# datastax/jvector

Measured on AMD Instinct MI355X. Metric: QPS@recall10>=0.95 (10Mx768); distances/sec as % HBM roofline, higher is better.
Workload: dtype f32

## Files before the change

### jvector_amd/csrc/cabi.cpp

```cpp
#include <algorithm>
#include <cmath>
#include <cstring>
#include <mutex>

#include "jv_device.h"
#include "jv_internal.h"
#include "gs_params.h"
#include "../../include/jvector_formats.h"

namespace jv {

static thread_local char g_err[1024] = "";

void set_error(const char *fmt, ...)
{
    va_list ap;
    va_start(ap, fmt);
    vsnprintf(g_err, sizeof(g_err), fmt, ap);
    va_end(ap);
}
void clear_error() { g_err[0] = 0; }

int Buffer::reserve(size_t bytes)
{
// ... 238 lines not shown
    ctx->d_gs_visited.release();
    ctx->d_gs_spill.release();
    ctx->d_gs_out.release();
    ctx->d_gs_mask.release();
    ctx->d_gs_big.release();
    ctx->d_nvq_q.release();
    ctx->d_gs_extra.release();
    ctx->d_gs_ubr.release();
    ctx->d_bq_work.release();
    ctx->d_bin_work.release();
    ctx->d_bin_cand.release();
    ctx->d_rd_counts.release();
    for (auto &e : ctx->prof_pending) {
        (void)hipEventDestroy(e.start);
        (void)hipEventDestroy(e.stop);
    }
    for (auto &e : ctx->prof_free) (void)hipEventDestroy(e);
    if (ctx->owns_stream) (void)hipStreamDestroy(ctx->stream);
    delete ctx;
    return JV_OK;
}

int jv_hip_ctx_sync(jv_ctx *ctx)
{
    JV_REQUIRE(ctx, "ctx is NULL");
    JV_HIP_CHECK(hipStreamSynchronize(ctx->stream));
    return JV_OK;
}

void *jv_hip_ctx_stream(jv_ctx *ctx) { return ctx ? (void *)ctx->stream : nullptr; }

static int prof_resolve(jv_ctx *ctx)
{
    if (ctx->prof_pending.empty()) return JV_OK;
    JV_HIP_CHECK(hipStreamSynchronize(ctx->stream));
    for (auto &e : ctx->prof_pending) {
        float ms = 0.0f;
        if (hipEventElapsedTime(&ms, e.start, e.stop) == hipSuccess) {
            ctx->prof_ms[e.region] += ms;
            ctx->prof_count[e.region] += 1;
        } else {
            (void)hipGetLastError();
        }
        ctx->prof_free.push_back(e.start);
        ctx->prof_free.push_back(e.stop);
    }
    ctx->prof_pending.clear();
    return JV_OK;
}

int jv_hip_ctx_profile(jv_ctx *ctx, int enable)
{
    clear_error();
    JV_REQUIRE(ctx, "ctx is NULL");
    JV_TRY(use_device(ctx->device));
    JV_TRY(prof_resolve(ctx));
    for (int r = 0; r < R_COUNT; ++r) {
        ctx->prof_ms[r] = 0.0;
        ctx->prof_count[r] = 0;
    }
    ctx->profiling = enable != 0;
    return JV_OK;
}

int jv_hip_ctx_profile_read(jv_ctx *ctx, const char *region, double *total_ms, int64_t *count)
{
    clear_error();
    JV_REQUIRE(ctx && region, "NULL argument");
    static const char *names[R_COUNT] = {"adc", "topk", "exact", "lut", "encode", "norms", "sample", "gsearch", "prune", "adc_exact"};
    int r = -1;
    for (int i = 0; i < R_COUNT; ++i)
        if (strcmp(names[i], region) == 0) r = i;
    JV_REQUIRE(r >= 0, "unknown profile region '%s'", region);
    JV_TRY(use_device(ctx->device));
    JV_TRY(prof_resolve(ctx));
    if (total_ms) *total_ms = ctx->prof_ms[r];
    if (count) *count = ctx->prof_count[r];
    return JV_OK;
}

}
namespace jv {
namespace {
const char *const kOptions[] = {"graph_traversal", "gs_occ", "gs_pair", "gs_pairc", "gs_quad", "rd_table_free", "rd_chunk", "rd_split", "rd_wide_stage", "rd_prof", "rd_square", "bl_insert_alpha_x100", "bl_improve_beam", "bl_ref_order", "bl_sorted_lists", "gs_cand_cap", "gs_waves_per_cu", "gs_vcap_log2", "gs_v1_log2", "gs_prefetch", "gs_generic", "gs_wgx", "gs_wgx_waves", "gs_wgx_slots", "gs_wgx_depth", "gs_wgx_per_cu", "gs_wgx_lut_m", "gs_ubr", "gs_ubrc", "gs_ubr_trim", "gs_plain", "gs_fused_rerank", "gs_defer", "gs_defer_min_level", "adc_bq",
                                "gs_grow", "gs_retry", "gs_prof", "gs_tie_check", "gs_push_log", "gs_push_log_cap", "graph_timing",
                                "no_filter", "quiet", "bq_gs_vcap_log2", "bq_gs_cand_cap", "flat_acc_score_bytes"};
std::string env_name(const char *name)
{
    std::string e = "JVECTOR_HIP_";
    for (const char *c = name; *c; ++c) e.push_back((char)toupper((unsigned char)*c));
    return e;
}
}
bool ctx_opt_is_set(const jv_ctx *ctx, const char *name)
{
    if (ctx && ctx->opts.count(name)) return true;
    return getenv(env_name(name).c_str()) != nullptr;
}
long long ctx_opt(const jv_ctx *ctx, const char *name, long long dflt)
{
    if (ctx) {
        auto it = ctx->opts.find(name);
        if (it != ctx->opts.end()) return it->second;
    }
    const char *e = getenv(env_name(name).c_str());
    if (!e) return dflt;
    if (!strcmp(name, "graph_traversal")) return !strcmp(e, "host") ? JV_TRAVERSAL_HOST : (!strcmp(e, "device") ? JV_TRAVERSAL_DEVICE : dflt);
    return atoll(e);
}
}
extern "C" {

int jv_hip_ctx_set_option(jv_ctx *ctx, const char *name, int64_t value)
{
    clear_error();
    JV_REQUIRE(ctx && name, "ctx_set_option: NULL argument");
    for (const char *k : kOptions)
        if (!strcmp(k, name)) {
            ctx->opts[name] = (long long)value;
            return JV_OK;
        }
    set_error("ctx_set_option: unknown option '%s'", name);
    return JV_ERR_INVALID;
}

int jv_hip_ctx_clear_option(jv_ctx *ctx, const char *name)
{
    clear_error();
    JV_REQUIRE(ctx && name, "ctx_clear_option: NULL argument");
    ctx->opts.erase(name);
    return JV_OK;
}

int jv_hip_ctx_get_stat(jv_ctx *ctx, const char *name, int64_t *out)
{
    clear_error();
    JV_REQUIRE(ctx && name && out, "ctx_get_stat: NULL argument");
    if (strcmp(name, "experimental_build") == 0) {
#ifdef JV_EXPERIMENTAL
        *out = 1;
#else
        *out = 0;
#endif
        return JV_OK;
    }
    if (strcmp(name, "rd_tests") == 0 || strcmp(name, "rd_pairs") == 0) {
        *out = 0;
        if (ctx->d_rd_counts.ptr) {
            unsigned long long h[2] = {0, 0};
            JV_TRY(use_device(ctx->device));
            JV_HIP_CHECK(hipStreamSynchronize(ctx->stream));
            JV_HIP_CHECK(hipMemcpy(h, ctx->d_rd_counts.ptr, sizeof(h), hipMemcpyDeviceToHost));
            *out = (int64_t)h[name[3] == 't' ? 0 : 1];
        }
        return JV_OK;
    }
    auto it = ctx->stats.find(name);
    *out = it == ctx->stats.end() ? 0 : (int64_t)it->second;
    return JV_OK;
}

int jv_hip_ctx_reset_stats(jv_ctx *ctx)
{
    clear_error();
    JV_REQUIRE(ctx, "ctx_reset_stats: NULL argument");
    ctx->stats.clear();
    return JV_OK;
// ... 1068 lines not shown
```

### jvector_amd/csrc/graph_search.cpp

```cpp
#include <algorithm>
#include <atomic>
#include <chrono>
#include <condition_variable>
#include <cstdlib>
#include <functional>
#include <memory>
#include <unordered_map>
#include <mutex>
#include <thread>

#include "gs_host.h"
#include "gs_params.h"
#include "jv_internal.h"

namespace jv {
constexpr long long kGsUbrDefault = 1;
constexpr long long kGsUbrcDefault = 1;


class HostPool {
public:
    explicit HostPool(int nthreads) : n_(nthreads)
    {
        for (int t = 1; t < n_; ++t) threads_.emplace_back([this, t] { worker(t); });
    }
    ~HostPool()
    {
        {
            std::lock_guard<std::mutex> lk(m_);
            stop_.store(true);
            awake_ = true;
        }
        cv_.notify_all();
        gen_.fetch_add(1, std::memory_order_release);
        for (auto &th : threads_) th.join();
    }
    int size() const { return n_; }
    void begin()
    {
        {
            std::lock_guard<std::mutex> lk(m_);
            awake_ = true;
        }
        cv_.notify_all();
    }
    void end()
    {
        std::lock_guard<std::mutex> lk(m_);
        awake_ = false;
    }
    void parallel_for(int n, const std::function<void(int, int)> &fn)
    {
        if (n_ == 1 || n < 2 * n_) {
            fn(0, n);
            return;
        }
        fn_ = &fn;
        total_ = n;
        done_.store(0, std::memory_order_relaxed);
        gen_.fetch_add(1, std::memory_order_release);
        run_chunk(0);
        while (done_.load(std::memory_order_acquire) != n_ - 1) cpu_relax();
    }

private:
    static inline void cpu_relax() { __builtin_ia32_pause(); }
    void run_chunk(int t)
    {
        const int per = (total_ + n_ - 1) / n_;
        const int lo = t * per, hi = std::min(total_, lo + per);
        if (lo < hi) (*fn_)(lo, hi);
    }
    void worker(int t)
    {
        uint64_t seen = 0;
        for (;;) {
            {
                std::unique_lock<std::mutex> lk(m_);
                cv_.wait(lk, [&] { return awake_ || stop_.load(); });
            }
            if (stop_.load()) return;
            long idle = 0;
            for (;;) {
                const uint64_t g = gen_.load(std::memory_order_acquire);
                if (g != seen) {
                    seen = g;
                    if (stop_.load()) return;
                    run_chunk(t);
                    done_.fetch_add(1, std::memory_order_release);
                    idle = 0;
                    continue;
                }
                cpu_relax();
                if (++idle > 4096) {
                    idle = 0;
                    bool aw;
// ... 1023 lines not shown

    return rerank_stage(ctx, pool, l, vectors, vsf, kvsf, Q, topK, opt, ses, fin, q_visited, q_expanded, q_expanded_base, out_ids, out_scores, stats);
}

static int ensure_device_graph(jv_ctx *ctx, jv_graph *g)
{
    std::lock_guard<std::mutex> lk(g->dev_mu);
    if (g->dev_ready) {
        JV_REQUIRE(g->dev_device == ctx->device, "graph: device mirror lives on device %d, search runs on device %d",
                   g->dev_device, ctx->device);
        return JV_OK;
    }
    g->free_mirror();
    g->dev_device = ctx->device;
    g->dev.resize((size_t)g->entry_level + 1);
    auto upload = [&](int32_t **dst, const int32_t *src, size_t n) -> int {
        JV_HIP_CHECK(hipMalloc((void **)dst, sizeof(int32_t) * std::max<size_t>(n, 1)));
        JV_HIP_CHECK(hipMemcpy(*dst, src, sizeof(int32_t) * n, hipMemcpyHostToDevice));
        return JV_OK;
    };
    auto build = [&]() -> int {
        for (int lv = 0; lv <= g->entry_level; ++lv) {
            const jv_graph::Level &L = g->levels[lv];
            jv_graph::DevLevel &d = g->dev[lv];
            if (lv == 0 && g->dev_level0) {
                d.nbrs = const_cast<int32_t *>(g->dev_level0);
                continue;
            }
            JV_TRY(upload(&d.nbrs, L.nbrs.data(), L.nbrs.size()));
            if (!L.nodes.empty()) {
                const GsLevelMap m = gs_build_level_map(L.nodes.data(), L.count);
                JV_TRY(upload(&d.hkeys, m.keys.data(), m.keys.size()));
                JV_TRY(upload(&d.hvals, m.vals.data(), m.vals.size()));
                d.hmask = m.mask;
                d.hshift = m.shift;
            }
        }
        return JV_OK;
    };
    const int rc = build();
    if (rc != JV_OK) {
        g->free_mirror();
        return rc;
    }
    g->dev_ready = true;
    return JV_OK;
}

extern "C++" {
namespace jv {
int graph_device_view(jv_ctx *ctx, const jv_graph *g, GsLevel *lv, GraphDeviceView *out)
{
    JV_REQUIRE(ctx && g && lv && out, "graph: NULL argument");
    JV_REQUIRE(g->entry_node >= 0, "graph: no entry node set");
    if (g->entry_level >= GS_MAX_LEVELS) {
        set_error("graph: %d levels, the device traversal takes %d", g->entry_level + 1, GS_MAX_LEVELS);
        return JV_ERR_UNSUPPORTED;
    }
    if (g->levels[0].nbrs.empty() && !g->dev_level0) {
        set_error("graph: level 0 has neither host rows nor a device adjacency");
        return JV_ERR_UNSUPPORTED;
    }
    JV_TRY(ensure_device_graph(ctx, const_cast<jv_graph *>(g)));
    out->n_nodes = g->n_nodes;
    out->entry_node = g->entry_node;
    out->entry_level = g->entry_level;
    out->max_degree = 0;
    for (int l = 0; l <= g->entry_level; ++l) {
        const jv_graph::DevLevel &d = g->dev[l];
        lv[l].nbrs = d.nbrs;
        lv[l].hkeys = d.hkeys;
        lv[l].hvals = d.hvals;
        lv[l].hmask = d.hmask;
        lv[l].hshift = d.hshift;
        lv[l].count = g->levels[l].count;
        lv[l].degree = g->levels[l].degree;
        out->max_degree = std::max(out->max_degree, g->levels[l].degree);
    }
    return JV_OK;
}
}
}

struct DeviceSessionOut {
    float threshold = 0.0f;
    const std::vector<jv_searcher::Call> *history = nullptr;
    int new_rerankK = 0;
    int log_cap = 0;
    std::vector<int32_t> status, base, log_n;
    std::vector<int64_t> stats;
    std::vector<long long> log;
};

static int graph_search_device(jv_ctx *ctx, const jv_graph *g, jv_luts *l, const jv_codes *codes, const jv_fused *fused,
                               const jv_vectors *vectors, const float *queries, int Q, jv_vsf vsf, int topK, int rerankK,
                               int32_t *out_ids, float *out_scores, int64_t *stats, AcceptMask host_accept, AcceptMask dev_accept,
                               DeviceSessionOut *so = nullptr)
{
    const jv_decoder_kind kind = fused ? JV_DECODER_FUSED : JV_DECODER_PQ;
    JV_TRY(luts_prepare(ctx, l, queries, Q, vsf, kind, false));
    const int kvsf = to_kernel_vsf(vsf);
    if (vsf == JV_COSINE) {
        JV_TRY(ensure_code_norms(ctx, const_cast<jv_codes *>(codes)));
        if (fused) JV_TRY(ensure_fused_norms(ctx, const_cast<jv_fused *>(fused)));
    }
    JV_TRY(ensure_device_graph(ctx, const_cast<jv_graph *>(g)));
    const jv_pq *pq = l->pq;

    const bool generic = !graph_search_device_specialised(pq, codes, fused) || ctx_opt(ctx, "gs_generic", 0) != 0;
    const int occ = ctx_opt(ctx, "gs_occ", generic ? 4 : 2) >= 4 ? 4 : 2;
    bool pair = occ == 2 && !generic && ctx_opt(ctx, "gs_pair", 1) != 0;
    for (int lv = 0; lv <= g->entry_level; ++lv) pair = pair && g->levels[lv].degree <= 32;
    pair = pair && pq->M <= 96;
    const long long wgx_opt = ctx_opt(ctx, "gs_wgx", -1);
    bool one_wave_tuned = false;
    for (const char *o : {"gs_vcap_log2", "gs_v1_log2", "gs_grow", "gs_retry", "gs_occ", "gs_pair", "gs_cand_cap", "gs_waves_per_cu", "gs_prefetch", "gs_prof"})
        one_wave_tuned = one_wave_tuned || ctx_opt_is_set(ctx, o);
    bool wgx = !so && !generic && graph_search_wgx_supported(pq->M) &&
               (wgx_opt > 0 || (wgx_opt < 0 && !one_wave_tuned && Q <= 4 * ctx->num_cus));
    for (int lv = 0; lv <= g->entry_level; ++lv) wgx = wgx && g->levels[lv].degree <= 64;
    const int wgx_log = std::min(512, std::max(256, 4 * rerankK));
    int wgx_kps = 32;
    for (int lv = 0; lv <= g->entry_level; ++lv)
        if (g->levels[lv].degree > 32) wgx_kps = 64;
    const int wgx_waves = std::max(2, std::min(8, (int)ctx_opt(ctx, "gs_wgx_waves", 8)));
    const int wgx_slots = std::max(2, std::min((int)GX_MAX_SLOTS, (int)ctx_opt(ctx, "gs_wgx_slots", 16)));
    int evict_cap = GS_EVICT_CAP;
    const int wgx_cand_cap = 256;
    const int wgx_per_cu = std::max(1, std::min(4, (int)ctx_opt(ctx, "gs_wgx_per_cu", 1)));
    const size_t wgx_budget = ctx->lds_per_block / (size_t)wgx_per_cu - (wgx_per_cu > 1 ? 256 : 512);
    auto wgx_bytes = [&](int lg, int lm) { return graph_search_wgx_lds_bytes(pq->D, rerankK, wgx_cand_cap, evict_cap, lg, wgx_slots, wgx_kps, wgx_log, lm); };
    int wgx_lut_m = (int)ctx_opt(ctx, "gs_wgx_lut_m", 0);
    if (wgx) {
        const int idb = gs_idbits(g->n_nodes);
        int min_v1 = 0;
        for (int lg = 12; lg >= 8 && min_v1 == 0; --lg)
            if (gs_v1_fits(lg, idb)) min_v1 = lg;
        if (wgx_lut_m <= 0) {
            wgx_lut_m = pq->M;
            while (wgx_lut_m > 16 && wgx_bytes(min_v1, wgx_lut_m) > wgx_budget) wgx_lut_m -= 16;
        }
        wgx_lut_m = std::max(16, std::min(pq->M, wgx_lut_m / 16 * 16));
        wgx = wgx_bytes(0, wgx_lut_m) <= wgx_budget;
    }
    if (wgx) pair = false;
    bool pairc = occ == 2 && !so && !wgx && !pair && !generic && !fused && pq->M <= 192 && ctx_opt(ctx, "gs_pair", 1) != 0 &&
                 ctx_opt(ctx, "gs_pairc", 1) != 0;
    for (int lv = 0; lv <= g->entry_level; ++lv) pairc = pairc && g->levels[lv].degree <= 64;
    const bool ubr = !so && !wgx && (pair || (pairc && ctx_opt(ctx, "gs_ubrc", kGsUbrcDefault) != 0)) && occ == 2 && !dev_accept.bits && !dev_accept.exclude &&
                     ctx_opt(ctx, "gs_ubr", kGsUbrDefault) != 0 && graph_search_ubr_supported(pq->M, kvsf)
#ifdef JV_EXPERIMENTAL
                     && ctx_opt(ctx, "gs_quad", 0) == 0
#endif
        ;
    const int pair_M = (pair || pairc) ? pq->M : 0;
    int cand_cap = wgx ? wgx_cand_cap : std::max(128, (int)ctx_opt(ctx, "gs_cand_cap", (occ == 4 ? 512 : ((pair || pairc) ? 256 : 1024)))) & ~63;
    while (!wgx && cand_cap > 256 && graph_search_lds_bytes(pq->D, rerankK, cand_cap, pair_M, evict_cap) > 40 * 1024) cand_cap = (cand_cap / 2) & ~63;
    const int idbits = gs_idbits(g->n_nodes);
    const int want_per_cu = 4 * occ;
    const size_t lut_lds = so ? gs_session_lds_bytes() : 0;
    const size_t lds_budget = (160 * 1024) / (size_t)want_per_cu - 256 - lut_lds;
    int v1_log2 = 0;
    if (wgx) {
        const long long pin = ctx_opt(ctx, "gs_v1_log2", ctx_opt_is_set(ctx, "gs_vcap_log2") ? 0 : -1);
        for (int lg = pin > 0 ? (int)pin : 14; lg >= (pin > 0 ? (int)pin : 8) && pin != 0; --lg) {
            if (!gs_v1_fits(lg, idbits)) continue;
            if (wgx_bytes(lg, wgx_lut_m) <= wgx_budget) {
                v1_log2 = lg;
                break;
            }
        }
    } else {
        const long long pin = ctx_opt(ctx, "gs_v1_log2", ctx_opt_is_set(ctx, "gs_vcap_log2") ? 0 : -1);
        struct Caps { int cand, evict; };
        const int cand_small = std::min(cand_cap, 128);
        const long long left = (long long)lds_budget - (long long)graph_search_lds_bytes(pq->D, rerankK, cand_small, pair_M, 1, 12) + 8;
        const Caps caps[3] = {{cand_cap, evict_cap}, {cand_small, evict_cap}, {cand_small, (int)std::max<long long>(96, std::min<long long>(evict_cap, left / 8))}};
        bool done = false;
        for (int lg = pin > 0 ? (int)pin : 12; lg >= (pin > 0 ? (int)pin : 10) && !done && pin != 0; --lg) {
            if (!gs_v1_fits(lg, idbits)) continue;
            for (const Caps &c : caps) {
                if (ctx_opt_is_set(ctx, "gs_cand_cap") && c.cand != cand_cap) continue;
                if (graph_search_lds_bytes(pq->D, rerankK, c.cand, pair_M, c.evict, lg) <= lds_budget || (pin > 0 && &c == &caps[2])) {
                    v1_log2 = lg;
                    cand_cap = c.cand;
                    evict_cap = c.evict;
                    done = true;
                    break;
                }
            }
        }
    }
    const size_t lds = wgx ? wgx_bytes(v1_log2, wgx_lut_m)
                           : graph_search_lds_bytes(pq->D, rerankK, cand_cap, pair_M, evict_cap, v1_log2) + lut_lds;
    if (lds > ctx->lds_per_block) {
        set_error("graph_search(device): rerankK %d needs %zu bytes of LDS per wave (limit %zu); use the host traversal", rerankK,
                  lds, ctx->lds_per_block);
        return JV_ERR_UNSUPPORTED;
    }
    int per_cu = (int)std::min<size_t>((size_t)want_per_cu, std::max<size_t>(1, (160 * 1024) / (lds + 256)));
    per_cu = std::max(1, (int)ctx_opt(ctx, "gs_waves_per_cu", per_cu));
    if (wgx) per_cu = wgx_per_cu;
    const int workers = std::max(1, std::min(Q, ctx->num_cus * per_cu));
    const int vcap_log2 = std::max(8, std::min(24, (int)ctx_opt(ctx, "gs_vcap_log2", gs_vcap_log2(rerankK))));
    const size_t vcap = (size_t)1 << vcap_log2;
    const size_t v1_slots = v1_log2 > 0 ? ((size_t)1 << v1_log2) : 0;
    const int spill_cap = (int)(vcap / 2 + v1_slots) + 64;
    JV_TRY(ctx->d_gs_visited.reserve(sizeof(int32_t) * vcap * (size_t)workers));
    JV_TRY(ctx->d_gs_spill.reserve(sizeof(long long) * (size_t)spill_cap * (size_t)workers));
    const int big_log2 = std::min(24, vcap_log2 + 3);
    const bool grow_on = ctx_opt_is_set(ctx, "gs_grow") ? ctx_opt(ctx, "gs_grow", 1) != 0 : !ctx_opt_is_set(ctx, "gs_vcap_log2");
    const int big_count = (grow_on && big_log2 > vcap_log2) ? std::max(1, std::min(Q, std::max(64, std::min(2048, Q / 32)))) : 0;
    const int big_spill_cap = (int)(((size_t)1 << big_log2) / 2 + v1_slots) + 64;
    const size_t big_vis_bytes = sizeof(int32_t) * ((size_t)1 << big_log2) * (size_t)big_count;
    const size_t big_spill_off = (big_vis_bytes + 255) & ~(size_t)255;
    const size_t big_ctr_off = (big_spill_off + sizeof(long long) * (size_t)big_spill_cap * (size_t)big_count + 255) & ~(size_t)255;
    if (big_count > 0) {
        JV_TRY(ctx->d_gs_big.reserve(big_ctr_off + 256));
        JV_HIP_CHECK(hipMemsetAsync((char *)ctx->d_gs_big.ptr + big_ctr_off, 0, sizeof(uint32_t), ctx->stream));
    }
    const size_t c1 = (size_t)Q * rerankK;
    size_t off = 0;
    auto carve = [&](size_t bytes) {
        const size_t o = off;
        off = (off + bytes + 255) & ~(size_t)255;
        return o;
    };
    const size_t o_ids = carve(sizeof(int32_t) * c1), o_sc = carve(sizeof(float) * c1), o_qn = carve(sizeof(float) * (size_t)Q);
    const size_t o_stats = carve(sizeof(long long) * 2 * (size_t)Q), o_status = carve(sizeof(int32_t) * (size_t)Q);
    const size_t o_counter = carve(sizeof(uint32_t) * 2);
    const size_t o_qmap = carve(sizeof(int32_t) * (size_t)Q);
    bool gs_prof = !so && ctx_opt(ctx, "gs_prof", 0) != 0;
    if (gs_prof && pairc) {
        if (ctx_opt(ctx, "quiet", 0) == 0)
            fprintf(stderr, "[jv gs prof] the compacted pair form (rows of 33..64 neighbours: the builder's searches) has no phase-clock variant; gs_prof ignored for this launch\n");
        gs_prof = false;
    }
    const size_t o_prof = carve(sizeof(unsigned long long) * 36);
    const bool defer_on = !so && !wgx && ubr && pair && ctx_opt(ctx, "gs_defer", 1) != 0 &&
                          (ctx_opt_is_set(ctx, "gs_defer") || g->defer_off.load(std::memory_order_relaxed) == 0);
    const bool tie_check = !so && vectors != nullptr && rerankK > topK && ctx_opt(ctx, "gs_tie_check", 1) != 0;
    int log_cap = 0;
    if (so || (tie_check && ctx_opt(ctx, "gs_push_log", 1) != 0)) {
        log_cap = so ? std::max(4096, 8 * rerankK) : std::max(256, 4 * rerankK);
        const size_t budget = (size_t)1 << 30;
        if ((size_t)Q * log_cap * sizeof(long long) > budget) log_cap = (int)std::max<size_t>(64, budget / ((size_t)Q * sizeof(long long)));
        if (ctx_opt_is_set(ctx, "gs_push_log_cap")) log_cap = std::max(1, (int)ctx_opt(ctx, "gs_push_log_cap", log_cap));
    }
    const size_t o_log = carve(sizeof(long long) * (size_t)Q * (size_t)log_cap), o_log_n = carve(sizeof(int32_t) * (size_t)Q);
    const size_t o_base = carve(sizeof(int32_t) * (size_t)Q);
    JV_TRY(ctx->d_gs_out.reserve(off));
    char *base = (char *)ctx->d_gs_out.ptr;
    int32_t *d_cand = (int32_t *)(base + o_ids);
    float *d_cand_sc = (float *)(base + o_sc);
    float *d_qnorm = (float *)(base + o_qn);
    long long *d_stats = (long long *)(base + o_stats);
    int32_t *d_status = (int32_t *)(base + o_status);
    uint32_t *d_counter = (uint32_t *)(base + o_counter);
    JV_HIP_CHECK(hipMemsetAsync(d_counter, 0, sizeof(uint32_t), ctx->stream));
    if (gs_prof || ubr) JV_HIP_CHECK(hipMemsetAsync(base + o_prof, 0, sizeof(unsigned long long) * 36, ctx->stream));

    GsParams p{};
    for (int lv = 0; lv <= g->entry_level; ++lv) {
        const jv_graph::DevLevel &d = g->dev[lv];
        p.lv[lv].nbrs = d.nbrs;
        p.lv[lv].hkeys = d.hkeys;
        p.lv[lv].hvals = d.hvals;
        p.lv[lv].hmask = d.hmask;
        p.lv[lv].hshift = d.hshift;
        p.lv[lv].count = g->levels[lv].count;
        p.lv[lv].degree = g->levels[lv].degree;
    }
    p.entry_node = g->entry_node;
    p.entry_level = g->entry_level;
    p.codebooks = pq->d_codebooks;
    p.cq = l->d_queries;
    p.bmag = l->d_bmag;
    p.codes = codes->d_codes;
    p.code_norms = codes->d_norms;
    p.blocks = fused ? fused->d_blocks : nullptr;
    p.fused_norms = fused ? fused->d_norms : nullptr;
    p.D = pq->D;
    p.M = pq->M;
    p.deg0 = g->levels[0].degree;
    p.generic = generic ? 1 : 0;
    p.sub_uniform4 = (generic && pq->uniform && pq->max_size % 4 == 0) ? pq->max_size : 0;
    p.sub_sizes = pq->d_sizes;
    p.sub_offsets = pq->d_offsets;
    p.cb_offsets = reinterpret_cast<const long long *>(pq->d_cb_offsets);
    p.Q = Q;
    p.rerankK = rerankK;
    p.accept = (const unsigned long long *)dev_accept.bits;
    p.accept_stride = dev_accept.stride_words;
    p.exclude = dev_accept.exclude;
    p.visited = (int32_t *)ctx->d_gs_visited.ptr;
    p.vcap_log2 = vcap_log2;
    p.spill = (long long *)ctx->d_gs_spill.ptr;
    p.spill_cap = spill_cap;
    p.cand_cap = cand_cap;
    p.evict_cap = evict_cap;
    p.v1_log2 = v1_log2;
    p.v1_idbits = idbits;
    p.prefetch = (ctx_opt(ctx, "gs_prefetch", 0) != 0 && evict_cap >= 48 && !generic) ? 1 : 0;
    if (ubr) {
        const size_t tab_bytes = (gs_ubr_tab_bytes(pq->M) * (size_t)Q + 255) & ~(size_t)255;
        JV_TRY(ctx->d_gs_ubr.reserve(tab_bytes + sizeof(float) * 4 * (size_t)Q));
        p.ubr = 1;
        p.ubr_tab = (const uint32_t *)ctx->d_gs_ubr.ptr;
        p.ubr_meta = (const float *)((const char *)ctx->d_gs_ubr.ptr + tab_bytes);
        p.ubr_trim = std::max(1, (int)ctx_opt(ctx, "gs_ubr_trim", 16));
        p.ubr_count = (unsigned long long *)(base + o_prof) + 15;
        ProfScope ps(ctx, R_LUT);
        JV_TRY(launch_ubr_tables(ctx->stream, kvsf, pq->d_codebooks, l->d_queries, Q, pq->M, (uint32_t *)ctx->d_gs_ubr.ptr,
                                 (float *)((char *)ctx->d_gs_ubr.ptr + tab_bytes)));
    }
    if (wgx) {
        p.prefetch = 0;
        p.wgx = 1;
        p.wgx_slots = wgx_slots;
        p.wgx_kps = wgx_kps;
        p.wgx_log = wgx_log;
        p.wgx_lut_m = wgx_lut_m;
        p.wgx_depth = (int)ctx_opt(ctx, "gs_wgx_depth", 1);
    }
    auto launch = [&](const GsParams &pp, int w) -> int {
        if (pp.ubr) return launch_graph_search_ubr(ctx->stream, kvsf, pp, w, lds);
        return wgx ? launch_graph_search_wgx(ctx->stream, kvsf, pp, w, 64 * wgx_waves) : launch_graph_search(ctx->stream, kvsf, pp, w, occ);
    };
    if (so) {
        p.session = 1;
        p.threshold = so->threshold;
        p.out_base = (int32_t *)(base + o_base);
        if (so->history && !so->history->empty()) {
            const std::vector<jv_searcher::Call> &h = *so->history;
            const int np = (int)h.size() + 1;
            std::vector<int32_t> off((size_t)(np - 1) * Q + 1);
            size_t total = 0;
            for (int t = 0; t < np - 1; ++t) {
                p.ph_rerankK[t] = h[(size_t)t].rerankK;
                p.ph_threshold[t] = h[(size_t)t].threshold;
                for (int q = 0; q < Q; ++q) {
                    off[(size_t)t * Q + q] = (int32_t)total;
                    total += (size_t)(h[(size_t)t].ev_off[(size_t)q + 1] - h[(size_t)t].ev_off[(size_t)q]);
                }
            }
            off.back() = (int32_t)total;
            p.ph_rerankK[np - 1] = so->new_rerankK;
            p.ph_threshold[np - 1] = so->threshold;
            p.n_phases = np;
            p.ph_Q = Q;
            const size_t off_bytes = (sizeof(int32_t) * off.size() + 15) & ~(size_t)15;
            JV_TRY(ctx->d_gs_extra.reserve(off_bytes + sizeof(long long) * std::max<size_t>(total, 1)));
            JV_HIP_CHECK(hipMemcpyAsync(ctx->d_gs_extra.ptr, off.data(), sizeof(int32_t) * off.size(), hipMemcpyHostToDevice, ctx->stream));
            size_t at = 0;
            for (int t = 0; t < np - 1; ++t) {
                const size_t n = h[(size_t)t].ev_keys.size();
                if (n) JV_HIP_CHECK(hipMemcpyAsync((char *)ctx->d_gs_extra.ptr + off_bytes + sizeof(long long) * at, h[(size_t)t].ev_keys.data(),
                                                   sizeof(long long) * n, hipMemcpyHostToDevice, ctx->stream));
                at += n;
            }
            JV_HIP_CHECK(hipStreamSynchronize(ctx->stream));
            p.ph_extra_off = (const int32_t *)ctx->d_gs_extra.ptr;
            p.ph_extra = (const long long *)((const char *)ctx->d_gs_extra.ptr + off_bytes);
        }
    }
    if (big_count > 0) {
        p.big_visited = (int32_t *)ctx->d_gs_big.ptr;
        p.big_spill = (long long *)((char *)ctx->d_gs_big.ptr + big_spill_off);
        p.big_next = (uint32_t *)((char *)ctx->d_gs_big.ptr + big_ctr_off);
        p.big_count = big_count;
        p.big_log2 = big_log2;
        p.big_spill_cap = big_spill_cap;
    }
    p.pair = pair ? 1 : (pairc ? 2 : 0);
#ifdef JV_EXPERIMENTAL
    p.quad = ctx_opt(ctx, "gs_quad", 0) != 0 ? 1 : 0;
#else
    p.quad = 0;
#endif
    p.out_ids = d_cand;
    p.out_scores = d_cand_sc;
    p.out_stats = d_stats;
    p.out_status = d_status;
    p.next_query = d_counter;
    if (log_cap > 0) {
        p.push_log = (long long *)(base + o_log);
        p.push_log_n = (int32_t *)(base + o_log_n);
        p.push_log_cap = log_cap;
    }
    p.prof = gs_prof ? (unsigned long long *)(base + o_prof) : nullptr;
    p.plain = ctx_opt(ctx, "gs_plain", 1) != 0 ? 1 : 0;
    if (defer_on) {
        p.defer = 1;
        p.defer_count = (unsigned long long *)(base + o_prof) + 33;
        p.defer_min_level = (int)std::max<long long>(1, ctx_opt(ctx, "gs_defer_min_level", 2));
    }
    int rr_rows = 0;
    if (!so && !wgx && ubr && pair && vectors && !vectors->nvq && vectors->D == pq->D && gs_rr_lds_bytes() <= lds && ctx_opt(ctx, "gs_fused_rerank", 1) != 0) {
        if (vsf == JV_COSINE) JV_TRY(ensure_vector_norms(ctx, const_cast<jv_vectors *>(vectors)));
        rr_rows = exact_fused_rows(vectors->d_vecs, vectors->D, l->d_raw_queries, Q, kvsf, rerankK, vectors->d_sqnorm);
    }
    if (rr_rows > 0) {
        if (vsf == JV_COSINE) {
            ProfScope ps(ctx, R_EXACT);
            JV_TRY(launch_query_sqnorms(ctx->stream, l->d_raw_queries, vectors->D, Q, d_qnorm));
        }
        p.rr_vecs = vectors->d_vecs;
        p.rr_queries = l->d_raw_queries;
        p.rr_qnorm = d_qnorm;
        p.rr_vnorm = vectors->d_sqnorm;
        p.rr_n = vectors->count;
        p.rr_rows = rr_rows;
    }
    {
        ProfScope ps(ctx, R_GSEARCH);
        JV_TRY(launch(p, workers));
    }
    std::vector<int32_t> status((size_t)Q);
    std::vector<int> redo;
    size_t n_overflow_first = 0;
    {
        JV_TRY(ctx->h_out.reserve(sizeof(int32_t) * (size_t)Q));
        JV_HIP_CHECK(hipMemcpyAsync(ctx->h_out.ptr, d_status, sizeof(int32_t) * (size_t)Q, hipMemcpyDeviceToHost, ctx->stream));
        unsigned long long ubr_dropped = 0;
        if (ubr) JV_HIP_CHECK(hipMemcpyAsync(&ubr_dropped, base + o_prof + 15 * sizeof(unsigned long long), sizeof(ubr_dropped), hipMemcpyDeviceToHost, ctx->stream));
        unsigned long long defer_counts[3] = {0, 0, 0};
        if (defer_on) JV_HIP_CHECK(hipMemcpyAsync(defer_counts, base + o_prof + 33 * sizeof(unsigned long long), sizeof(defer_counts), hipMemcpyDeviceToHost, ctx->stream));
        JV_HIP_CHECK(hipStreamSynchronize(ctx->stream));
        if (ubr) ctx_stat_add(ctx, "gs_ubr_dropped", (long long)ubr_dropped);
        if (defer_on) {
            ctx_stat_add(ctx, "gs_deferred", (long long)defer_counts[0]);
            ctx_stat_add(ctx, "gs_defer_restarts", (long long)defer_counts[1]);
            if (Q >= 64 && defer_counts[1] * 10 > (unsigned long long)Q && g->defer_off.exchange(1, std::memory_order_relaxed) == 0)
                ctx_stat_add(ctx, "gs_defer_switched_off", 1);
        }
        memcpy(status.data(), ctx->h_out.ptr, sizeof(int32_t) * (size_t)Q);
        for (int q = 0; q < Q; ++q)
            if (status[q] != GS_OK) redo.push_back(q);
        n_overflow_first = redo.size();
    }
    const bool retry = ctx_opt_is_set(ctx, "gs_retry") ? ctx_opt(ctx, "gs_retry", 1) != 0 : !ctx_opt_is_set(ctx, "gs_vcap_log2");
    for (int attempt = 1; attempt <= 2 && !redo.empty() && retry; ++attempt) {
        const int vlog2 = std::min(24, vcap_log2 + 3 * attempt);
        if (vlog2 <= vcap_log2 + 3 * (attempt - 1)) break;
        const size_t vcap2 = (size_t)1 << vlog2;
        const int spill2 = (int)(vcap2 / 2 + v1_slots) + 64;
        const int R = (int)redo.size();
        const int workers2 = std::max(1, std::min<int>({R, workers, (int)(((size_t)512 << 20) / (vcap2 * 12))}));
        JV_TRY(ctx->d_gs_visited.reserve(sizeof(int32_t) * vcap2 * (size_t)workers2));
        JV_TRY(ctx->d_gs_spill.reserve(sizeof(long long) * (size_t)spill2 * (size_t)workers2));
        memcpy(ctx->h_out.ptr, redo.data(), sizeof(int32_t) * (size_t)R);
        JV_HIP_CHECK(hipMemcpyAsync(base + o_qmap, ctx->h_out.ptr, sizeof(int32_t) * (size_t)R, hipMemcpyHostToDevice, ctx->stream));
        JV_HIP_CHECK(hipMemsetAsync(d_counter, 0, sizeof(uint32_t), ctx->stream));
        GsParams p2 = p;
        p2.qmap = (const int32_t *)(base + o_qmap);
        p2.Q = R;
        p2.visited = (int32_t *)ctx->d_gs_visited.ptr;
        p2.vcap_log2 = vlog2;
        p2.spill = (long long *)ctx->d_gs_spill.ptr;
        p2.spill_cap = spill2;
        p2.big_visited = nullptr;
        p2.big_count = 0;
        p2.big_log2 = 0;
        p2.prof = nullptr;
        p2.defer = 0;
        {
            ProfScope ps(ctx, R_GSEARCH);
            JV_TRY(launch(p2, workers2));
        }
        JV_HIP_CHECK(hipStreamSynchronize(ctx->stream));
        JV_HIP_CHECK(hipMemcpyAsync(ctx->h_out.ptr, d_status, sizeof(int32_t) * (size_t)Q, hipMemcpyDeviceToHost, ctx->stream));
        JV_HIP_CHECK(hipStreamSynchronize(ctx->stream));
        memcpy(status.data(), ctx->h_out.ptr, sizeof(int32_t) * (size_t)Q);
        std::vector<int> still;
        for (int q : redo)
            if (status[q] != GS_OK) still.push_back(q);
        redo.swap(still);
    }
    if (gs_prof) {
        unsigned long long h[33];
        JV_HIP_CHECK(hipMemcpyAsync(h, base + o_prof, sizeof(h), hipMemcpyDeviceToHost, ctx->stream));
        JV_HIP_CHECK(hipStreamSynchronize(ctx->stream));
        const double e = (double)std::max<unsigned long long>(h[5], 1);
        fprintf(stderr, "[jv gs prof] clocks/expansion: pop %.0f  result %.0f  row+block+visited %.0f  score %.0f  push %.0f | expansions %llu "
                        "queries %llu  setup+epilogue clocks/query %.0f\n", h[0] / e, h[1] / e, h[2] / e, h[3] / e, h[4] / e, h[5], h[6],
                (double)h[7] / (double)std::max<unsigned long long>(h[6], 1));
        const double fs = (double)std::max<unsigned long long>(h[8] + h[9] + h[10] + h[11], 1);
        {
            const double nq = (double)std::max<unsigned long long>(h[6], 1);
            fprintf(stderr, "[jv gs prof] clocks/query outside the expansion loop: setup %.0f  level transitions %.0f  epilogue %.0f  table build %.0f\n",
                    h[12] / nq, h[13] / nq, h[14] / nq, h[15] / nq);
            fprintf(stderr, "[jv gs prof] levels above 0: %.2f expansions per query, %.0f clocks per query (searchOneLayer + transitions) = %.0f per expansion\n",
                    h[24] / nq, h[25] / nq, (double)h[25] / (double)std::max<unsigned long long>(h[24], 1));
            {
                const double eu = (double)std::max<unsigned long long>(h[24], 1);
                fprintf(stderr, "[jv gs prof] levels above 0, clocks/expansion: pop %.0f  result %.0f  row+visited %.0f  score %.0f  push %.0f | scoring passes %.2f per expansion, %.0f clocks per pass\n",
                        h[26] / eu, h[27] / eu, h[28] / eu, h[29] / eu, h[30] / eu, h[32] / eu, (double)h[31] / (double)std::max<unsigned long long>(h[32], 1));
            }
        }
        if (wgx)
            fprintf(stderr, "[jv gs prof] workgroup form, per expansion: row found in a slot %.3f (of those still being scored at use: %.3f of all)  "
                            "requested at the pop %.3f  rows requested ahead %.3f\n", h[8] / e, h[9] / e, h[10] / e, h[11] / e);
        else if (ubr) {
            fprintf(stderr, "[jv gs prof] register-table bound form, per expansion: bound + staging %.0f clocks  bound + staging + exact scores %.0f clocks  "
                            "trims %.0f clocks | dropped %.2f  exactly scored %.2f neighbours\n", h[8] / e, h[9] / e, h[10] / e, h[15] / e, h[11] / e);
            fprintf(stderr, "[jv gs prof] register-table bound form, per expansion: wait for the row %.0f clocks  scoring rounds %.0f  owner sum + finish %.0f  "
                            "passes %.2f | expansions with <= 4 / <= 8 / <= 16 survivors: %.3f / %.3f / %.3f\n", h[16] / e, h[17] / e, h[18] / e, h[19] / e,
                    h[20] / e, h[21] / e, h[22] / e);
        }
        else
        fprintf(stderr, "[jv gs prof] scored neighbours by fresh count of their expansion: <=8 %.3f  <=16 %.3f  <=24 %.3f  <=32 %.3f\n", h[8] / fs,
                h[9] / fs, h[10] / fs, h[11] / fs);
    }

    if (so) {
        so->status.assign(status.begin(), status.end());
        so->base.resize((size_t)Q);
        so->log_n.resize((size_t)Q);
        so->stats.resize(2 * (size_t)Q);
        JV_HIP_CHECK(hipMemcpyAsync(so->base.data(), base + o_base, sizeof(int32_t) * (size_t)Q, hipMemcpyDeviceToHost, ctx->stream));
        JV_HIP_CHECK(hipMemcpyAsync(so->log_n.data(), base + o_log_n, sizeof(int32_t) * (size_t)Q, hipMemcpyDeviceToHost, ctx->stream));
        JV_HIP_CHECK(hipMemcpyAsync(so->stats.data(), d_stats, sizeof(long long) * 2 * (size_t)Q, hipMemcpyDeviceToHost, ctx->stream));
        JV_HIP_CHECK(hipStreamSynchronize(ctx->stream));
        int longest = 0;
        bool overflowed = false;
        for (int q = 0; q < Q; ++q) {
            overflowed = overflowed || so->log_n[(size_t)q] > log_cap;
            longest = std::max(longest, std::min(so->log_n[(size_t)q], log_cap));
        }
        so->log_cap = overflowed ? -1 : std::max(longest, 1);
        if (!overflowed) {
            so->log.resize((size_t)Q * (size_t)so->log_cap);
            JV_HIP_CHECK(hipMemcpy2DAsync(so->log.data(), sizeof(long long) * (size_t)so->log_cap, base + o_log, sizeof(long long) * (size_t)log_cap,
                                          sizeof(long long) * (size_t)so->log_cap, (size_t)Q, hipMemcpyDeviceToHost, ctx->stream));
            JV_HIP_CHECK(hipStreamSynchronize(ctx->stream));
        }
        ctx_stat_add(ctx, "gs_calls_device", 1);
        ctx_stat_add(ctx, "gs_queries_device", Q);
        ctx_stat_add(ctx, "gs_session_calls_device", 1);
        return JV_OK;
    }
    OutStage oi, osc;
    JV_TRY(stage_out_begin(ctx, out_ids, sizeof(int32_t) * (size_t)Q * topK, ctx->d_scratch2, &oi));
    JV_TRY(stage_out_begin(ctx, out_scores, sizeof(float) * (size_t)Q * topK, ctx->d_scratch3, &osc));
    JV_TRY(ctx->d_scratch.reserve(topk_scratch_bytes(Q, topK)));
    if (vectors && rr_rows > 0) {
        if (rr_rows < rerankK) {
            ProfScope ps(ctx, R_EXACT);
            JV_TRY(launch_exact_gather_tail(ctx->stream, vectors->d_vecs, vectors->count, vectors->D, l->d_raw_queries, Q, kvsf, d_cand, rerankK, rr_rows,
                                            d_cand_sc, d_qnorm, vectors->d_sqnorm));
        }
    } else if (vectors) {
        JV_TRY(rerank_gather(ctx, vectors, l->d_raw_queries, Q, vsf, d_cand, rerankK, d_cand_sc, d_qnorm));
    }
    {
        ProfScope ps(ctx, R_TOPK);
        JV_TRY(launch_topk(ctx->stream, ctx, d_cand_sc, d_cand, Q, rerankK, rerankK, 0, topK, (int32_t *)oi.dev,
                           (float *)osc.dev, ctx->d_scratch.ptr));
    }
    if (tie_check) {
        JV_HIP_CHECK(hipMemsetAsync(d_counter, 0, sizeof(uint32_t) * 2, ctx->stream));
        ProfScope ps(ctx, R_TOPK);
        RtParams rt{};
        rt.cand_sc = d_cand_sc;
        rt.cand_ids = d_cand;
        rt.R = rerankK;
        rt.out_sc = (float *)osc.dev;
        rt.out_ids = (int32_t *)oi.dev;
        rt.K = topK;
        rt.Q = Q;
        rt.push_log = p.push_log;
        rt.push_log_n = p.push_log_n;
        rt.log_cap = p.push_log_cap;
        rt.rerankK = rerankK;
        rt.status = d_status;
        rt.count = d_counter;
        JV_TRY(launch_rerank_ties(ctx->stream, rt));
    }
    JV_TRY(stage_out_end(ctx, oi));
    JV_TRY(stage_out_end(ctx, osc));
    const size_t stats_bytes = stats ? sizeof(long long) * 2 * (size_t)Q : 0;
    JV_TRY(ctx->h_out.reserve(stats_bytes + 64));
    unsigned int *h_ties = (unsigned int *)((char *)ctx->h_out.ptr + stats_bytes);
    h_ties[0] = h_ties[1] = 0;
    if (tie_check) JV_HIP_CHECK(hipMemcpyAsync(h_ties, d_counter, sizeof(uint32_t) * 2, hipMemcpyDeviceToHost, ctx->stream));
    if (stats) {
        long long *h_stats = (long long *)ctx->h_out.ptr;
        JV_HIP_CHECK(hipMemcpyAsync(h_stats, d_stats, sizeof(long long) * 2 * (size_t)Q, hipMemcpyDeviceToHost, ctx->stream));
        JV_HIP_CHECK(hipStreamSynchronize(ctx->stream));
        for (int q = 0; q < Q; ++q) {
            stats[2 * q] = h_stats[2 * q];
            stats[2 * q + 1] = h_stats[2 * q + 1];
        }
    } else {
        JV_HIP_CHECK(hipStreamSynchronize(ctx->stream));
    }
    const size_t n_ties = h_ties[0], n_ties_resolved = h_ties[1];
    if (n_ties > 0) {
        JV_TRY(ctx->h_out.reserve(sizeof(int32_t) * (size_t)Q));
        JV_HIP_CHECK(hipMemcpyAsync(ctx->h_out.ptr, d_status, sizeof(int32_t) * (size_t)Q, hipMemcpyDeviceToHost, ctx->stream));
        JV_HIP_CHECK(hipStreamSynchronize(ctx->stream));
        const int32_t *hs = (const int32_t *)ctx->h_out.ptr;
        for (int q = 0; q < Q; ++q)
            if (hs[q] == GS_RERANK_TIE) redo.push_back(q);
        std::sort(redo.begin(), redo.end());
    }
    ctx_stat_add(ctx, "gs_calls_device", 1);
    ctx_stat_add(ctx, "gs_queries_device", Q);
    ctx_stat_add(ctx, "gs_queries_retried", (long long)n_overflow_first);
    ctx_stat_add(ctx, "gs_ties_resolved_device", (long long)n_ties_resolved);
    ctx_stat_add(ctx, "gs_ties_to_host", (long long)n_ties);
    ctx_stat_add(ctx, "gs_queries_host_fallback", (long long)redo.size());
    ctx_stat_set(ctx, "gs_last_v1_log2", v1_log2);
    ctx_stat_set(ctx, "gs_last_workers_per_cu", per_cu);
    ctx_stat_set(ctx, "gs_last_wgx", wgx ? 1 : 0);
    ctx_stat_set(ctx, "gs_last_ubr", ubr ? 1 : 0);
    ctx_stat_set(ctx, "gs_last_plain", (!wgx && gs_params_plain(p)) ? 1 : 0);
    ctx_stat_set(ctx, "gs_last_rr_rows", rr_rows);
    ctx_stat_set(ctx, "gs_last_pair", pair ? 1 : (pairc ? 2 : 0));
    if (wgx) ctx_stat_add(ctx, "gs_calls_wgx", 1);
    if (ctx_opt(ctx, "graph_timing", 0) != 0)
        fprintf(stderr, "[jv graph_search device] Q=%d workers=%d (x%d/CU, occ %d, pair %d, wgx %d) lds=%zu cand_cap=%d evict_cap=%d v1_log2=%d vcap=%zu overflow=%zu rerank ties=%zu (+%zu to the host) -> host %zu\n", Q,
                workers, per_cu, occ, pair ? 1 : (pairc ? 2 : 0), wgx ? wgx_waves : 0, lds, cand_cap, evict_cap, v1_log2, vcap, n_overflow_first, n_ties_resolved, n_ties, redo.size());
    if (redo.empty()) return JV_OK;

    jv_graph *gm = const_cast<jv_graph *>(g);
    std::unique_lock<std::mutex> loan_lock(gm->dev_mu, std::defer_lock);
    if (g->dev_level0) loan_lock.lock();
    struct Level0Loan {
        jv_graph *g;
        bool active = false;
        ~Level0Loan()
        {
            if (active) {
                g->levels[0].nbrs.clear();
                g->levels[0].nbrs.shrink_to_fit();
// ... 475 lines not shown
```

Baseline: 2.587 million.

## Add lean query preamble kernel replacing LUT preparation in device graph search

Adds a new HIP kernel that, in one pass over the raw queries, writes centered queries, computes per-query centered magnitudes for cosine, and optionally computes query squared norms. Device graph search uses it by default instead of the full luts_prepare path, stages host queries straight to the device, and reuses the kernel-computed query norms so the separate sqnorm launch is skipped. This targets per-call host and device preamble overhead, at the cost of a new code path that marks tables invalid and must match the old preparation exactly.

```diff
diff --git a/jvector_amd/csrc/cabi.cpp b/jvector_amd/csrc/cabi.cpp
--- a/jvector_amd/csrc/cabi.cpp
+++ b/jvector_amd/csrc/cabi.cpp
@@ -344,7 +344,7 @@
 }
 namespace jv {
 namespace {
-const char *const kOptions[] = {"graph_traversal", "gs_occ", "gs_pair", "gs_pairc", "gs_quad", "rd_table_free", "rd_chunk", "rd_split", "rd_wide_stage", "rd_prof", "rd_square", "bl_insert_alpha_x100", "bl_improve_beam", "bl_ref_order", "bl_sorted_lists", "gs_cand_cap", "gs_waves_per_cu", "gs_vcap_log2", "gs_v1_log2", "gs_prefetch", "gs_generic", "gs_wgx", "gs_wgx_waves", "gs_wgx_slots", "gs_wgx_depth", "gs_wgx_per_cu", "gs_wgx_lut_m", "gs_ubr", "gs_ubrc", "gs_ubr_trim", "gs_plain", "gs_fused_rerank", "gs_defer", "gs_defer_min_level", "adc_bq",
+const char *const kOptions[] = {"graph_traversal", "gs_occ", "gs_pair", "gs_pairc", "gs_quad", "rd_table_free", "rd_chunk", "rd_split", "rd_wide_stage", "rd_prof", "rd_square", "bl_insert_alpha_x100", "bl_improve_beam", "bl_ref_order", "bl_sorted_lists", "gs_cand_cap", "gs_waves_per_cu", "gs_vcap_log2", "gs_v1_log2", "gs_prefetch", "gs_generic", "gs_wgx", "gs_wgx_waves", "gs_wgx_slots", "gs_wgx_depth", "gs_wgx_per_cu", "gs_wgx_lut_m", "gs_ubr", "gs_ubrc", "gs_ubr_trim", "gs_plain", "gs_lean_step", "gs_fused_rerank", "gs_defer", "gs_defer_min_level", "adc_bq",
                                 "gs_grow", "gs_retry", "gs_prof", "gs_tie_check", "gs_push_log", "gs_push_log_cap", "graph_timing",
                                 "no_filter", "quiet", "bq_gs_vcap_log2", "bq_gs_cand_cap", "flat_acc_score_bytes"};
 std::string env_name(const char *name)
diff --git a/jvector_amd/csrc/graph_search.cpp b/jvector_amd/csrc/graph_search.cpp
--- a/jvector_amd/csrc/graph_search.cpp
+++ b/jvector_amd/csrc/graph_search.cpp
@@ -12,6 +12,7 @@
 #include "gs_host.h"
 #include "gs_params.h"
 #include "jv_internal.h"
+#include "sp_params.h"
 
 namespace jv {
 constexpr long long kGsUbrDefault = 1;
@@ -1201,6 +1202,49 @@
 }
 }
 
+extern "C++" {
+namespace jv {
+#ifdef __HIP__
+int launch_step_preamble(hipStream_t s, const SpPreParams &p, size_t p_bytes);
+static inline bool step_preamble_present() { return true; }
+#else
+int launch_step_preamble_emulated(hipStream_t s, const SpPreParams &p, size_t p_bytes) __attribute__((weak));
+static inline int launch_step_preamble(hipStream_t s, const SpPreParams &p, size_t p_bytes) { return launch_step_preamble_emulated(s, p, p_bytes); }
+static inline bool step_preamble_present() { return launch_step_preamble_emulated != nullptr; }
+#endif
+}
+}
+
+static int step_stage_queries(jv_ctx *ctx, jv_luts *l, const float *queries, int Q, jv_vsf vsf, jv_decoder_kind kind, const float **raw_out)
+{
+    *raw_out = nullptr;
+    if (!step_preamble_present()) return JV_OK;
+    if (!ctx || !l || !queries || Q <= 0 || Q > l->capacity) return JV_OK;
+    if (vsf != JV_EUCLIDEAN && vsf != JV_DOT_PRODUCT && vsf != JV_COSINE) return JV_OK;
+    const jv_pq *pq = l->pq;
+    if (pq->D < 8 || pq->D % 8 != 0) return JV_OK;
+    const bool block8 = kind != JV_DECODER_FUSED || (pq->uniform && pq->max_size == 8 && pq->D == 8 * pq->M);
+    if (vsf == JV_COSINE && !block8) return JV_OK;
+    const bool dev = is_device_ptr(queries);
+    if (dev && (reinterpret_cast<uintptr_t>(queries) & 15) != 0) return JV_OK;
+    JV_TRY(use_device(ctx->device));
+    l->Q = Q;
+    l->vsf = vsf;
+    l->kind = kind;
+    l->tables_valid = false;
+    if (dev) {
+        *raw_out = queries;
+        return JV_OK;
+    }
+    const size_t qbytes = sizeof(float) * (size_t)Q * pq->D;
+    JV_HIP_CHECK(hipStreamSynchronize(ctx->stream));
+    JV_TRY(ctx->h_in.reserve(qbytes));
+    memcpy(ctx->h_in.ptr, queries, qbytes);
+    JV_HIP_CHECK(hipMemcpyAsync(l->d_raw_queries, ctx->h_in.ptr, qbytes, hipMemcpyHostToDevice, ctx->stream));
+    *raw_out = l->d_raw_queries;
+    return JV_OK;
+}
+
 struct DeviceSessionOut {
     float threshold = 0.0f;
     const std::vector<jv_searcher::Call> *history = nullptr;
@@ -1217,7 +1261,14 @@
                                DeviceSessionOut *so = nullptr)
 {
     const jv_decoder_kind kind = fused ? JV_DECODER_FUSED : JV_DECODER_PQ;
-    JV_TRY(luts_prepare(ctx, l, queries, Q, vsf, kind, false));
+    const float *q_raw = nullptr;
+    if (!so && ctx_opt(ctx, "gs_lean_step", 1) != 0) JV_TRY(step_stage_queries(ctx, l, queries, Q, vsf, kind, &q_raw));
+    const bool lean_pre = q_raw != nullptr;
+    if (!lean_pre) {
+        JV_TRY(luts_prepare(ctx, l, queries, Q, vsf, kind, false));
+        q_raw = l->d_raw_queries;
+    }
+    ctx_stat_set(ctx, "gs_last_lean_step", lean_pre ? 1 : 0);
     const int kvsf = to_kernel_vsf(vsf);
     if (vsf == JV_COSINE) {
         JV_TRY(ensure_code_norms(ctx, const_cast<jv_codes *>(codes)));
@@ -1378,6 +1429,23 @@
     uint32_t *d_counter = (uint32_t *)(base + o_counter);
     JV_HIP_CHECK(hipMemsetAsync(d_counter, 0, sizeof(uint32_t), ctx->stream));
     if (gs_prof || ubr) JV_HIP_CHECK(hipMemsetAsync(base + o_prof, 0, sizeof(unsigned long long) * 36, ctx->stream));
+    const bool pre_qnorm = lean_pre && vsf == JV_COSINE && vectors && vectors->D == l->pq->D;
+    if (lean_pre) {
+        ProfScope ps(ctx, R_LUT);
+        SpPreParams sp{};
+        sp.raw = q_raw;
+        sp.centroid = l->pq->d_centroid;
+        sp.cq = l->d_queries;
+        sp.bmag = vsf == JV_COSINE ? l->d_bmag : nullptr;
+        sp.qnorm = pre_qnorm ? d_qnorm : nullptr;
+        sp.Q = Q;
+        sp.D = l->pq->D;
+        const int rc = launch_step_preamble(ctx->stream, sp, sizeof(sp));
+        if (rc != JV_OK) {
+            set_error("graph_search(device): the query preamble kernel could not be launched (%d)", rc);
+            return rc;
+        }
+    }
 
     GsParams p{};
     for (int lv = 0; lv <= g->entry_level; ++lv) {
@@ -1517,15 +1585,15 @@
     int rr_rows = 0;
     if (!so && !wgx && ubr && pair && vectors && !vectors->nvq && vectors->D == pq->D && gs_rr_lds_bytes() <= lds && ctx_opt(ctx, "gs_fused_rerank", 1) != 0) {
         if (vsf == JV_COSINE) JV_TRY(ensure_vector_norms(ctx, const_cast<jv_vectors *>(vectors)));
-        rr_rows = exact_fused_rows(vectors->d_vecs, vectors->D, l->d_raw_queries, Q, kvsf, rerankK, vectors->d_sqnorm);
+        rr_rows = exact_fused_rows(vectors->d_vecs, vectors->D, q_raw, Q, kvsf, rerankK, vectors->d_sqnorm);
     }
     if (rr_rows > 0) {
-        if (vsf == JV_COSINE) {
+        if (vsf == JV_COSINE && !pre_qnorm) {
             ProfScope ps(ctx, R_EXACT);
-            JV_TRY(launch_query_sqnorms(ctx->stream, l->d_raw_queries, vectors->D, Q, d_qnorm));
+            JV_TRY(launch_query_sqnorms(ctx->stream, q_raw, vectors->D, Q, d_qnorm));
         }
         p.rr_vecs = vectors->d_vecs;
-        p.rr_queries = l->d_raw_queries;
+        p.rr_queries = q_raw;
         p.rr_qnorm = d_qnorm;
         p.rr_vnorm = vectors->d_sqnorm;
         p.rr_n = vectors->count;
@@ -1666,11 +1734,11 @@
     if (vectors && rr_rows > 0) {
         if (rr_rows < rerankK) {
             ProfScope ps(ctx, R_EXACT);
-            JV_TRY(launch_exact_gather_tail(ctx->stream, vectors->d_vecs, vectors->count, vectors->D, l->d_raw_queries, Q, kvsf, d_cand, rerankK, rr_rows,
+            JV_TRY(launch_exact_gather_tail(ctx->stream, vectors->d_vecs, vectors->count, vectors->D, q_raw, Q, kvsf, d_cand, rerankK, rr_rows,
                                             d_cand_sc, d_qnorm, vectors->d_sqnorm));
         }
     } else if (vectors) {
-        JV_TRY(rerank_gather(ctx, vectors, l->d_raw_queries, Q, vsf, d_cand, rerankK, d_cand_sc, d_qnorm));
+        JV_TRY(rerank_gather(ctx, vectors, q_raw, Q, vsf, d_cand, rerankK, d_cand_sc, d_qnorm));
     }
     {
         ProfScope ps(ctx, R_TOPK);
diff --git a/jvector_amd/csrc/k_step.hip b/jvector_amd/csrc/k_step.hip
--- /dev/null
+++ b/jvector_amd/csrc/k_step.hip
@@ -0,0 +1,37 @@
+#include <hip/hip_runtime.h>
+
+#include <cstddef>
+#include <cstdint>
+
+#include "../../include/jvector_hip.h"
+#include "sp_params.h"
+
+#include "gs_wave_hip.h"
+
+#include "sp_body.h"
+
+#define SP_EXPORT __attribute__((visibility("default")))
+
+namespace jv {
+
+template <bool CENTER>
+__global__ __launch_bounds__(64) void step_preamble_kernel(SpPreParams p)
+{
+    __shared__ __attribute__((aligned(16))) float tile[(SP_ROWS + 1) * SP_LS];
+    sp_preamble<CENTER>(p, (int64_t)blockIdx.x, tile);
+}
+
+SP_EXPORT int launch_step_preamble(hipStream_t s, const SpPreParams &p, size_t p_bytes)
+{
+    if (p_bytes != sizeof(SpPreParams) || p.Q < 0 || !p.raw || !p.cq || p.raw == p.cq) return JV_ERR_INVALID;
+    if (p.Q == 0) return JV_OK;
+    const uintptr_t align = reinterpret_cast<uintptr_t>(p.raw) | reinterpret_cast<uintptr_t>(p.cq) | reinterpret_cast<uintptr_t>(p.centroid);
+    if (p.D < 8 || p.D % 8 != 0 || (align & 15) != 0) return JV_ERR_UNSUPPORTED;
+    const dim3 grid((unsigned)((p.Q + SP_ROWS - 1) / SP_ROWS));
+    if (p.centroid) hipLaunchKernelGGL(step_preamble_kernel<true>, grid, dim3(64), 0, s, p);
+    else hipLaunchKernelGGL(step_preamble_kernel<false>, grid, dim3(64), 0, s, p);
+    if (hipGetLastError() != hipSuccess) return JV_ERR_HIP;
+    return JV_OK;
+}
+
+}
diff --git a/jvector_amd/csrc/sp_body.h b/jvector_amd/csrc/sp_body.h
--- /dev/null
+++ b/jvector_amd/csrc/sp_body.h
@@ -0,0 +1,86 @@
+#pragma once
+
+#include <cstdint>
+
+#include "sp_params.h"
+
+namespace jv {
+
+template <bool CENTER>
+GS_FN void sp_preamble(const SpPreParams &p, int64_t wave, float *tile )
+{
+    constexpr int CH = SP_CH, LS = SP_LS;
+    const int lane = gs_lane();
+    const int seg = (lane & 15) * 4;
+    const int sub = lane >> 4;
+    const int64_t q0 = wave * SP_ROWS;
+    const int D = p.D;
+    const int nc = (D + CH - 1) / CH;
+    SpF4 r[16], cen{0.0f, 0.0f, 0.0f, 0.0f};
+    auto issue = [&](int c) {
+        const int col = c * CH + seg < D ? c * CH + seg : 0;
+#pragma unroll
+        for (int k = 0; k < 16; ++k) {
+            const int64_t q = q0 + 4 * k + sub < p.Q ? q0 + 4 * k + sub : (int64_t)p.Q - 1;
+            r[k] = *reinterpret_cast<const SpF4 *>(p.raw + q * D + col);
+        }
+        if (CENTER) cen = *reinterpret_cast<const SpF4 *>(p.centroid + col);
+    };
+    issue(0);
+    float mag = 0.0f, nrm = 0.0f;
+    for (int c = 0; c < nc; ++c) {
+        const bool in = c * CH + seg < D;
+#pragma unroll
+        for (int k = 0; k < 16; ++k) {
+            *reinterpret_cast<SpF4 *>(tile + (4 * k + sub) * LS + seg) = r[k];
+            const int64_t q = q0 + 4 * k + sub;
+            if (q < p.Q && in) {
+                SpF4 o{r[k].x, r[k].y, r[k].z, r[k].w};
+                if (CENTER) {
+                    o.x = o.x - cen.x;
+                    o.y = o.y - cen.y;
+                    o.z = o.z - cen.z;
+                    o.w = o.w - cen.w;
+                }
+                *reinterpret_cast<SpF4 *>(p.cq + q * D + c * CH + seg) = o;
+            }
+        }
+        if (CENTER && sub == 0) *reinterpret_cast<SpF4 *>(tile + SP_ROWS * LS + seg) = cen;
+        gs_barrier();
+        if (c + 1 < nc) issue(c + 1);
+        const int len = (D - c * CH < CH) ? (D - c * CH) : CH;
+        const float *row = tile + lane * LS;
+        const float *cn = tile + SP_ROWS * LS;
+        for (int i = 0; i < len; i += 8) {
+            const SpF4 v0 = *reinterpret_cast<const SpF4 *>(row + i), v1 = *reinterpret_cast<const SpF4 *>(row + i + 4);
+            if (p.qnorm) {
+                nrm += v0.x * v0.x; nrm += v0.y * v0.y; nrm += v0.z * v0.z; nrm += v0.w * v0.w;
+                nrm += v1.x * v1.x; nrm += v1.y * v1.y; nrm += v1.z * v1.z; nrm += v1.w * v1.w;
+            }
+            if (p.bmag) {
+                float e0 = v0.x, e1 = v0.y, e2 = v0.z, e3 = v0.w, e4 = v1.x, e5 = v1.y, e6 = v1.z, e7 = v1.w;
+                if (CENTER) {
+                    const SpF4 c0 = *reinterpret_cast<const SpF4 *>(cn + i), c1 = *reinterpret_cast<const SpF4 *>(cn + i + 4);
+                    e0 = e0 - c0.x; e1 = e1 - c0.y; e2 = e2 - c0.z; e3 = e3 - c0.w;
+                    e4 = e4 - c1.x; e5 = e5 - c1.y; e6 = e6 - c1.z; e7 = e7 - c1.w;
+                }
+                float t = e0 * e0 + e1 * e1;
+                t = t + e2 * e2;
+                t = t + e3 * e3;
+                t = t + e4 * e4;
+                t = t + e5 * e5;
+                t = t + e6 * e6;
+                t = t + e7 * e7;
+                mag += t;
+            }
+        }
+        gs_barrier();
+    }
+    const int64_t q = q0 + lane;
+    if (q < p.Q) {
+        if (p.bmag) p.bmag[q] = mag;
+        if (p.qnorm) p.qnorm[q] = nrm;
+    }
+}
+
+}
diff --git a/jvector_amd/csrc/sp_params.h b/jvector_amd/csrc/sp_params.h
--- /dev/null
+++ b/jvector_amd/csrc/sp_params.h
@@ -0,0 +1,27 @@
+#pragma once
+
+#include <cstddef>
+#include <cstdint>
+
+namespace jv {
+
+constexpr int SP_CH = 64;
+constexpr int SP_LS = SP_CH + 4;
+constexpr int SP_ROWS = 64;
+
+struct alignas(16) SpF4 {
+    float x, y, z, w;
+};
+
+struct SpPreParams {
+    const float *raw;
+    const float *centroid;
+    float *cq;
+    float *bmag;
+    float *qnorm;
+    int Q, D;
+};
+
+constexpr size_t sp_pre_lds_bytes() { return sizeof(float) * (SP_ROWS + 1) * SP_LS; }
+
+}
```

Result: no change. 2.613 million, median of 6 (+1.0%).
